# eridgd/WCT-TF

Measured on AMD Instinct MI355X. Metric: stylized frames/sec @512x512, 5-level relu5->1 pipeline, alpha=0.8, higher is better.
Workload: dtype f16

## Files before the change

wct_tf_amd/csrc/stats_gemm.hip:

```cpp
#include "wct_stages.h"


struct StatArgs {
  const float* x[2];
  int n[2];
  const float* u[2];
  const unsigned* umax[2];
  const float* mean;
  float* partial;
  float* absmax;
  int C, nslab;
  int shared_style;
};

__global__ __launch_bounds__(256) void colsum_kernel(StatArgs p) {
  __shared__ f32x4 red[256];
  const int mat = blockIdx.y, slab = blockIdx.x;
  if (skip_style_mat(mat, p.shared_style)) return;
  const int b = mat & 1, pair = mat >> 1;
  const int C = p.C, cq = C / 4;
  const int nrp = 256 / cq;
  const int tid = threadIdx.x;
  const int rp = tid / cq, c4 = tid % cq;
  const int N = p.n[b];
// ... 367 lines not shown
#pragma unroll
      for (int i = 0; i < TM; ++i)
#pragma unroll
        for (int j = 0; j < TM; ++j) {
          acc[i][j] = __builtin_amdgcn_mfma_f32_32x32x16_f16(al[i], bhf[j], acc[i][j], 0, 0, 0);
          acc[i][j] = __builtin_amdgcn_mfma_f32_32x32x16_f16(ah[i], blf[j], acc[i][j], 0, 0, 0);
          acc[i][j] = __builtin_amdgcn_mfma_f32_32x32x16_f16(ah[i], bhf[j], acc[i][j], 0, 0, 0);
        }
    }
  };

  float ra[KPT], rb[KPT];
  if (diag) {
    if (kbeg < kend) load(ra, voff_a, kbeg);
    for (int k0 = kbeg; k0 < kend; k0 += 32) {
      if (k0 + 32 <= kend) split_store(ra, mean_a, k0, false, lds[0], lds[1]);
      else split_store(ra, mean_a, k0, true, lds[0], lds[1]);
      __syncthreads();
      if (k0 + 32 < kend) load(ra, voff_a, k0 + 32);
      mma_stage(lds[0], lds[1]);
      __syncthreads();
    }
  } else {
    if (kbeg < kend) { load(ra, voff_a, kbeg); load(rb, voff_b, kbeg); }
    for (int k0 = kbeg; k0 < kend; k0 += 32) {
      if (k0 + 32 <= kend) {
        split_store(ra, mean_a, k0, false, lds[0], lds[1]);
        split_store(rb, mean_b, k0, false, lds[2], lds[3]);
      } else {
        split_store(ra, mean_a, k0, true, lds[0], lds[1]);
        split_store(rb, mean_b, k0, true, lds[2], lds[3]);
      }
      __syncthreads();
      if (k0 + 32 < kend) { load(ra, voff_a, k0 + 32); load(rb, voff_b, k0 + 32); }
      mma_stage(lds[2], lds[3]);
      __syncthreads();
    }
  }

  float* out = p.partial + ((size_t)mat * p.nsplit + split) * C * C;
#pragma unroll
  for (int i = 0; i < TM; ++i)
#pragma unroll
    for (int j = 0; j < TM; ++j) {
      const int gn = n0 + (wn * TM + j) * 32 + (lane & 31);
#pragma unroll
      for (int r = 0; r < 16; ++r) {
        const int gm = m0 + (wm * TM + i) * 32 + (r & 3) + 8 * (r >> 2) + 4 * (lane >> 5);
        if (gm < C && gn < C) out[(size_t)gm * C + gn] = acc[i][j][r];
      }
    }
}

__global__ __launch_bounds__(256) void cov_finish_kernel(const float* partial, const float* scale, float* cov, int C, int nsplit, int BT,
                                                         float inv0, float inv1, float eps, int shared_style, float* cov0 = nullptr) {
  __shared__ float tt[64][65];
  const int mat = blockIdx.z;
  if (skip_style_mat(mat, shared_style)) return;
  const size_t cc = (size_t)C * C;
  const int r0 = blockIdx.y * 64, c0 = blockIdx.x * 64, tid = threadIdx.x, ty = tid >> 4, tx = tid & 15;
  const bool mirror = r0 / BT > c0 / BT;
  const float* pb = partial + (size_t)mat * nsplit * cc;
  const float sc = scale[mat];
  const float f = ((mat & 1) == 0 ? inv0 : inv1) / (sc * sc);
  f32x4 acc[4];
#pragma unroll
  for (int i = 0; i < 4; ++i) {
    const int r = (mirror ? c0 : r0) + ty * 4 + i, c = (mirror ? r0 : c0) + tx * 4;
    f32x4 sum = {0.f, 0.f, 0.f, 0.f};
    if (r < C && c < C)
      for (int k = 0; k < nsplit; ++k) sum += *reinterpret_cast<const f32x4*>(pb + (size_t)k * cc + (size_t)r * C + c);
    acc[i] = sum;
  }
  if (mirror) {
#pragma unroll
    for (int i = 0; i < 4; ++i)
#pragma unroll
      for (int j = 0; j < 4; ++j) tt[ty * 4 + i][tx * 4 + j] = acc[i][j];
    __syncthreads();
#pragma unroll
    for (int i = 0; i < 4; ++i)
#pragma unroll
      for (int j = 0; j < 4; ++j) acc[i][j] = tt[tx * 4 + j][ty * 4 + i];
  }
#pragma unroll
  for (int i = 0; i < 4; ++i) {
    const int r = r0 + ty * 4 + i, c = c0 + tx * 4;
    if (r >= C || c >= C) continue;
    f32x4 v = acc[i] * f;
#pragma unroll
    for (int j = 0; j < 4; ++j) if (r == c + j) v[j] += eps;
    *reinterpret_cast<f32x4*>(cov + (size_t)mat * cc + (size_t)r * C + c) = v;
    if (cov0) *reinterpret_cast<f32x4*>(cov0 + (size_t)mat * cc + (size_t)r * C + c) = v;
  }
}

int launch_means(const float* content, int Nc, const float* style, int Ns, int C, int P,
                        const WctCarve& w, bool with_var, int shared_style, hipStream_t s, const WctFeatStats* fs) {
  StatArgs sa;
  sa.x[0] = content; sa.x[1] = style; sa.n[0] = Nc; sa.n[1] = Ns;
  for (int b = 0; b < 2; ++b) {
    sa.u[b] = fs && fs->umax[b] ? fs->u[b] : nullptr;
    sa.umax[b] = sa.u[b] ? fs->umax[b] : nullptr;
  }
  sa.mean = nullptr; sa.partial = w.stat_partial; sa.absmax = w.absmax; sa.C = C; sa.nslab = w.nslab; sa.shared_style = shared_style;
  hipLaunchKernelGGL(colsum_kernel, dim3(w.nslab, 2 * P), dim3(256), 0, s, sa);
  hipLaunchKernelGGL(colsum_finish_kernel, dim3(cdiv(C, 256), 2 * P), dim3(256), 0, s, w.stat_partial, w.mean, C, w.nslab, (float)Nc, (float)Ns, shared_style,
                     (const float*)w.absmax, w.scale);
  if (with_var) {
    sa.mean = w.mean; sa.absmax = nullptr;
    hipLaunchKernelGGL(colsum_kernel, dim3(w.nslab, 2 * P), dim3(256), 0, s, sa);
    hipLaunchKernelGGL(colsum_finish_kernel, dim3(cdiv(C, 256), 2 * P), dim3(256), 0, s, w.stat_partial, w.var, C, w.nslab, (float)Nc, (float)Ns, shared_style,
                       (const float*)nullptr, (float*)nullptr);
  }
  HIP_TRY(hipGetLastError());
  return WCT_OK;
}

int launch_cov(const float* content, int Nc, const float* style, int Ns, int C, int P, const WctCarve& w, float eps, int shared_style,
               hipStream_t s) {
  const int BT = C >= 128 ? 128 : 64;
  {
    CovArgs ca;
    ca.x[0] = content; ca.x[1] = style; ca.n[0] = Nc; ca.n[1] = Ns;
    ca.mean = w.mean; ca.scale = w.scale; ca.partial = w.cov_partial;
    ca.C = C; ca.ksplit = w.ksplit; ca.nsplit = w.nsplit; ca.ntile = cdiv(C, BT); ca.shared_style = shared_style;
    dim3 grid(ca.ntile * (ca.ntile + 1) / 2, w.nsplit, 2 * P);
    if (BT == 128) hipLaunchKernelGGL((cov_f16x2_kernel<128>), grid, dim3(256), 0, s, ca);
    else hipLaunchKernelGGL((cov_f16x2_kernel<64>), grid, dim3(256), 0, s, ca);
    HIP_TRY(hipGetLastError());
  }
  hipLaunchKernelGGL(cov_finish_kernel, dim3(cdiv(C, 64), cdiv(C, 64), 2 * P), dim3(256), 0, s, w.cov_partial, w.scale, w.A, C,
                     w.nsplit, BT, 1.f / (float)(Nc - 1), 1.f / (float)(Ns - 1), eps, shared_style, w.A0);
  HIP_TRY(hipGetLastError());
  return WCT_OK;
}

static int launch_slot_means(const float* x, int N, int C, int m, int nslab, const WctCarve& w, bool with_var, hipStream_t s,
                             const float* u = nullptr, const unsigned* umax = nullptr) {
  StatArgs sa = {};
  sa.x[0] = sa.x[1] = x; sa.n[0] = sa.n[1] = N;
  sa.u[0] = umax ? u : nullptr; sa.umax[0] = sa.u[0] ? umax : nullptr;
  float* partial = w.stat_partial + (size_t)m * w.nslab * C;
  float* absmax = w.absmax + (size_t)m * w.nslab;
  sa.mean = nullptr; sa.partial = partial; sa.absmax = absmax; sa.C = C; sa.nslab = nslab; sa.shared_style = 0;
  hipLaunchKernelGGL(colsum_kernel, dim3(nslab, 1), dim3(256), 0, s, sa);
  hipLaunchKernelGGL(colsum_finish_kernel, dim3(cdiv(C, 256), 1), dim3(256), 0, s, partial, w.mean + (size_t)m * C, C, nslab, (float)N,
                     (float)N, 0, (const float*)absmax, w.scale + m);
  if (with_var) {
    sa.mean = w.mean + (size_t)m * C; sa.absmax = nullptr;
    hipLaunchKernelGGL(colsum_kernel, dim3(nslab, 1), dim3(256), 0, s, sa);
    hipLaunchKernelGGL(colsum_finish_kernel, dim3(cdiv(C, 256), 1), dim3(256), 0, s, partial, w.var + (size_t)m * C, C, nslab, (float)N,
                       (float)N, 0, (const float*)nullptr, (float*)nullptr);
  }
  HIP_TRY(hipGetLastError());
  return WCT_OK;
}

static int launch_slot_cov(const float* x, int N, int C, int m, int nsplit, int ksplit, float eps, const WctCarve& w, hipStream_t s) {
  const int BT = C >= 128 ? 128 : 64;
  const size_t cc = (size_t)C * C;
  CovArgs ca;
  ca.x[0] = ca.x[1] = x; ca.n[0] = ca.n[1] = N;
  ca.mean = w.mean + (size_t)m * C; ca.scale = w.scale + m; ca.partial = w.cov_partial + (size_t)m * w.nsplit * cc;
  ca.C = C; ca.ksplit = ksplit; ca.nsplit = nsplit; ca.ntile = cdiv(C, BT); ca.shared_style = 0;
  dim3 grid(ca.ntile * (ca.ntile + 1) / 2, nsplit, 1);
  if (BT == 128) hipLaunchKernelGGL((cov_f16x2_kernel<128>), grid, dim3(256), 0, s, ca);
  else hipLaunchKernelGGL((cov_f16x2_kernel<64>), grid, dim3(256), 0, s, ca);
  hipLaunchKernelGGL(cov_finish_kernel, dim3(cdiv(C, 64), cdiv(C, 64), 1), dim3(256), 0, s,
                     ca.partial, ca.scale, w.A + m * cc, C, nsplit, BT, 1.f / (float)(N - 1), 1.f / (float)(N - 1), eps, 0, w.A0 + m * cc);
  HIP_TRY(hipGetLastError());
  return WCT_OK;
}

int launch_plan_stats(const SlotPlan& sp, int C, bool with_var, bool with_cov, float eps, hipStream_t s) {
  int rc;
  for (int m = 0; m < 2 * sp.P; ++m) {
    const SlotPlan::Slot& t = sp.slot[m];
    if (!t.n) continue;
    if ((rc = launch_slot_means(t.x, t.n, C, m, t.lay.nslab, sp.w, with_var, s, m ? nullptr : sp.u0, m ? nullptr : sp.umax0))) return rc;
    if (with_cov && (rc = launch_slot_cov(t.x, t.n, C, m, t.lay.nsplit, t.lay.ksplit, eps, sp.w, s))) return rc;
  }
  return WCT_OK;
}
```

wct_tf_amd/csrc/wct.hip:

```cpp
#include "wct_stages.h"
#include "jacobi_dev.h"
#include <algorithm>
#include <type_traits>



template <int BC, int BP, typename Args = ApplyArgs>
__global__ __launch_bounds__(256, 2) void apply_f16x2_kernel(Args p) {
  constexpr bool SEGB = std::is_same<Args, ApplySegBatchArgs>::value;
  constexpr bool SEG = std::is_same<Args, ApplySegArgs>::value || SEGB;
  constexpr int TM = BC / 64, TN = BP / 64;
  constexpr int MI = BC * 4 / 256, XI = BP * 4 / 256;
  __shared__ __attribute__((aligned(16))) unsigned char lm[2][BC * 64];
  __shared__ __attribute__((aligned(16))) unsigned char lx[2][BP * 64];
  typedef unsigned int u32x4 __attribute__((ext_vector_type(4)));
  const int tid = threadIdx.x, lane = tid & 63, wave = tid >> 6;
  const int wm = wave >> 1, wn = wave & 1;
  const int pair = blockIdx.z;
  const int n0 = blockIdx.x * BP, c0 = blockIdx.y * BC;
  int seg0 = 0, N = p.N;
  [[maybe_unused]] int row0 = 0;
  if constexpr (SEGB) {
    const int f = seg_frame(p.fl[pair]), lab = seg_label(p.fl[pair]);
    const int first = p.seg_off[f * (WCT_MIX_MAX + 1) + lab];
    N = p.seg_off[f * (WCT_MIX_MAX + 1) + lab + 1] - first;
    if (n0 >= N) return;
    row0 = f * p.N;
    seg0 = row0 + first;
  } else if constexpr (SEG) {
    seg0 = p.seg_off[p.lab[pair]];
    N = p.seg_off[p.lab[pair] + 1] - seg0;
    if (n0 >= N) return;
  }
  const int C = p.C;
  const float* x = p.x + (SEG ? (size_t)seg0 * C : (size_t)pair * N * C);
  const float* M = p.M + (size_t)pair * C * C;
  const float* mean = p.mean + (size_t)pair * 2 * C;
  const float sx = p.xscale[2 * pair];
  float sM = 1.f;
  {
    const float m = __uint_as_float(p.mabs[pair]);
    if (m > 0.f) { int e; frexpf(m, &e); sM = ldexpf(1.f, 14 - e); }
  }

  const float* mp[MI]; const float* xp[XI];
  int moff[MI], xoff[XI], xk[XI];
#pragma unroll
  for (int i = 0; i < MI; ++i) {
    const int item = tid + i * 256, row = item >> 2, kq = item & 3;
    mp[i] = M + (size_t)min(c0 + row, C - 1) * C + kq * 8;
    moff[i] = (row * 4 + (kq ^ ((row >> 2) & 3))) * 16;
  }
#pragma unroll
  for (int i = 0; i < XI; ++i) {
    const int item = tid + i * 256, row = item >> 2, kq = item & 3;
    xp[i] = x + (size_t)min(n0 + row, N - 1) * C + kq * 8;
    xoff[i] = (row * 4 + (kq ^ ((row >> 2) & 3))) * 16;
    xk[i] = kq * 8;
  }

  f32x16 acc[TM][TN];
#pragma unroll
  for (int i = 0; i < TM; ++i)
#pragma unroll
    for (int j = 0; j < TN; ++j)
#pragma unroll
      for (int r = 0; r < 16; ++r) acc[i][j][r] = 0.f;

  f32x4 rm[MI][2], rx[XI][2];
  auto load = [&](int k0) {
#pragma unroll
    for (int i = 0; i < MI; ++i) {
      rm[i][0] = *reinterpret_cast<const f32x4*>(mp[i] + k0);
      rm[i][1] = *reinterpret_cast<const f32x4*>(mp[i] + k0 + 4);
    }
#pragma unroll
    for (int i = 0; i < XI; ++i) {
      rx[i][0] = *reinterpret_cast<const f32x4*>(xp[i] + k0) - *reinterpret_cast<const f32x4*>(mean + k0 + xk[i]);
      rx[i][1] = *reinterpret_cast<const f32x4*>(xp[i] + k0 + 4) - *reinterpret_cast<const f32x4*>(mean + k0 + xk[i] + 4);
    }
  };
  auto split_store = [&](const f32x4 (&r)[2], float sc, unsigned char* hi, unsigned char* lo, int off) {
    half8 h, l;
#pragma unroll
    for (int j = 0; j < 8; ++j) {
      const float v = r[j >> 2][j & 3] * sc;
      h[j] = (half_t)v;
      l[j] = (half_t)(v - (float)h[j]);
    }
    *reinterpret_cast<half8*>(hi + off) = h;
    *reinterpret_cast<half8*>(lo + off) = l;
  };

  load(0);
  for (int k0 = 0; k0 < C; k0 += 32) {
#pragma unroll
    for (int i = 0; i < MI; ++i) split_store(rm[i], sM, lm[0], lm[1], moff[i]);
#pragma unroll
    for (int i = 0; i < XI; ++i) split_store(rx[i], sx, lx[0], lx[1], xoff[i]);
    __syncthreads();
    if (k0 + 32 < C) load(k0 + 32);
#pragma unroll
    for (int ks = 0; ks < 2; ++ks) {
      const int chunk = ks * 2 + (lane >> 5);
      half8 ah[TM], al[TM], bh[TN], bl[TN];
#pragma unroll
      for (int i = 0; i < TM; ++i) {
        const int r = (wm * TM + i) * 32 + (lane & 31);
        const int off = (r * 4 + (chunk ^ ((r >> 2) & 3))) * 16;
        ah[i] = *reinterpret_cast<const half8*>(lm[0] + off);
        al[i] = *reinterpret_cast<const half8*>(lm[1] + off);
      }
#pragma unroll
      for (int j = 0; j < TN; ++j) {
        const int r = (wn * TN + j) * 32 + (lane & 31);
        const int off = (r * 4 + (chunk ^ ((r >> 2) & 3))) * 16;
        bh[j] = *reinterpret_cast<const half8*>(lx[0] + off);
        bl[j] = *reinterpret_cast<const half8*>(lx[1] + off);
      }
#pragma unroll
      for (int i = 0; i < TM; ++i)
#pragma unroll
        for (int j = 0; j < TN; ++j) {
          acc[i][j] = __builtin_amdgcn_mfma_f32_32x32x16_f16(al[i], bh[j], acc[i][j], 0, 0, 0);
          acc[i][j] = __builtin_amdgcn_mfma_f32_32x32x16_f16(ah[i], bl[j], acc[i][j], 0, 0, 0);
          acc[i][j] = __builtin_amdgcn_mfma_f32_32x32x16_f16(ah[i], bh[j], acc[i][j], 0, 0, 0);
        }
    }
    __syncthreads();
  }

  const float inv = 1.f / (sx * sM);
  const float* bias = p.bias + (size_t)pair * C;
  const int kgrp = lane >> 5;
  f32x4 bvs[TM][4];
#pragma unroll
  for (int i = 0; i < TM; ++i)
#pragma unroll
    for (int rq = 0; rq < 4; ++rq) {
      const int co = c0 + (wm * TM + i) * 32 + 8 * rq + 4 * kgrp;
      const f32x4 z = {0.f, 0.f, 0.f, 0.f};
      bvs[i][rq] = co < C ? *reinterpret_cast<const f32x4*>(bias + co) : z;
    }
  int dst[TN];
  if constexpr (SEG)
#pragma unroll
    for (int j = 0; j < TN; ++j) {
      const int n = n0 + (wn * TN + j) * 32 + (lane & 31);
      dst[j] = p.perm[seg0 + (n < N ? n : 0)];
      if constexpr (SEGB) dst[j] += row0;
    }
#pragma unroll
  for (int j = 0; j < TN; ++j) {
    const int n = n0 + (wn * TN + j) * 32 + (lane & 31);
    const bool n_ok = n < N;
    const size_t row = SEG ? (size_t)dst[j] * C : ((size_t)pair * N + (n_ok ? n : 0)) * C;
#pragma unroll
    for (int i = 0; i < TM; ++i) {
      const int cb = c0 + (wm * TM + i) * 32;
      unsigned pk[4][2];
#pragma unroll
      for (int rq = 0; rq < 4; ++rq) {
        const int co = cb + 8 * rq + 4 * kgrp;
        const f32x4 bv = bvs[i][rq];
        f32x4 v;
#pragma unroll
        for (int q = 0; q < 4; ++q) v[q] = acc[i][j][rq * 4 + q] * inv + bv[q];
        if (p.out32 && n_ok && co < C) *reinterpret_cast<f32x4*>(p.out32 + row + co) = v;
        typedef _Float16 h2 __attribute__((ext_vector_type(2)));
        h2 lo = {(half_t)v[0], (half_t)v[1]}, hi = {(half_t)v[2], (half_t)v[3]};
        pk[rq][0] = __builtin_bit_cast(unsigned, lo);
        pk[rq][1] = __builtin_bit_cast(unsigned, hi);
      }
      if (p.out16) {
#pragma unroll
        for (int m = 0; m < 2; ++m) {
          auto sxw = __builtin_amdgcn_permlane32_swap(pk[2 * m][0], pk[2 * m + 1][0], false, false);
          auto syw = __builtin_amdgcn_permlane32_swap(pk[2 * m][1], pk[2 * m + 1][1], false, false);
          u32x4 o = {sxw[0], syw[0], sxw[1], syw[1]};
          const int co = cb + 16 * m + 8 * kgrp;
          if (n_ok && co < C) *reinterpret_cast<u32x4*>(p.out16 + row + co) = o;
        }
      }
    }
  }
}

int launch_apply_seg(const ApplySegArgs& a, int nmax, int P, hipStream_t s) {
  const int C = a.C;
  if (C >= 128) hipLaunchKernelGGL((apply_f16x2_kernel<128, 128, ApplySegArgs>), dim3(cdiv(nmax, 128), cdiv(C, 128), P), dim3(256), 0, s, a);
  else hipLaunchKernelGGL((apply_f16x2_kernel<64, 128, ApplySegArgs>), dim3(cdiv(nmax, 128), cdiv(C, 64), P), dim3(256), 0, s, a);
  HIP_TRY(hipGetLastError());
  return WCT_OK;
}

int launch_apply_seg_batch(const ApplySegBatchArgs& a, int nmax, int P, hipStream_t s) {
  const int C = a.C;
  if (C >= 128) hipLaunchKernelGGL((apply_f16x2_kernel<128, 128, ApplySegBatchArgs>), dim3(cdiv(nmax, 128), cdiv(C, 128), P), dim3(256), 0, s, a);
  else hipLaunchKernelGGL((apply_f16x2_kernel<64, 128, ApplySegBatchArgs>), dim3(cdiv(nmax, 128), cdiv(C, 64), P), dim3(256), 0, s, a);
  HIP_TRY(hipGetLastError());
  return WCT_OK;
}

static int wct_nslab(int N) { int s = cdiv(N, 64); return s < 1 ? 1 : (s > 256 ? 256 : s); }

static void cov_split(int C, int Nmax, int P, int* nsplit, int* ksplit) {
  const int nt = C >= 128 ? cdiv(C, 128) : 1;
  const int tiles = nt * (nt + 1) / 2 * P;
  int want = 32 / tiles;
  if (want < 1) want = 1;
  int ks = cdiv(cdiv(Nmax, want), 32) * 32;
  if (ks < 256) ks = 256;
  *ksplit = ks;
  *nsplit = cdiv(Nmax, ks);
}

PairLayout pair_layout(int C, int Nc, int Ns) {
  PairLayout L;
  const int Nmax = Nc > Ns ? Nc : Ns;
  L.nslab = wct_nslab(Nmax);
  cov_split(C, Nmax, 1, &L.nsplit, &L.ksplit);
  return L;
}

WctCarve carve(void* base, int C, int P, const PairLayout& lay) {
  WctCarve w;
  w.nslab = lay.nslab; w.nsplit = lay.nsplit; w.ksplit = lay.ksplit;
  size_t off = 0;
  char* b = reinterpret_cast<char*>(base);
  auto take = [&](size_t bytes) { void* p = b ? b + off : nullptr; off += align_up(bytes); return p; };
  const size_t cc = (size_t)C * C * sizeof(float);
  w.mean = (float*)take((size_t)2 * P * C * sizeof(float));
  w.var = (float*)take((size_t)2 * P * C * sizeof(float));
  w.stat_partial = (float*)take((size_t)2 * P * w.nslab * C * sizeof(float));
  w.absmax = (float*)take((size_t)2 * P * w.nslab * sizeof(float));
  w.scale = (float*)take((size_t)2 * P * sizeof(float));
  w.cov_partial = (float*)take((size_t)2 * P * w.nsplit * cc);
  w.A = (float*)take(2 * P * cc);
  w.A0 = (float*)take(2 * P * cc);
  w.refresh = (int*)take((size_t)2 * P * sizeof(int));
  w.V = (float*)take(2 * P * cc);
  w.d = (float*)take((size_t)2 * P * C * sizeof(float));
  w.G = (float*)take(2 * P * cc);
  w.X = (float*)take(2 * P * cc);
  w.S2 = (float*)take(7 * P * cc);
  w.Tw = (float*)take(2 * P * cc);
  w.Tcs = w.Tw + (size_t)C * C;
  w.T = (float*)take(P * cc);
  w.M = (float*)take(P * cc);
  w.bias = (float*)take((size_t)P * C * sizeof(float));
  w.mabs = (unsigned*)take((size_t)P * sizeof(unsigned));
  w.jacobi_bytes = jacobi_workspace_bytes(C, 2 * P) + 4 * (1024 + 64 * sizeof(JacobiState));
  w.jacobi_ws = take(w.jacobi_bytes);
  w.mix = (float*)take((size_t)2 * C * sizeof(float));
  w.total = off;
  return w;
}

size_t wct_workspace_bytes(int C, int Nc, int Ns, int P) {
  const int Cw = C < 32 ? 32 : C;
  return carve(nullptr, Cw, P, pair_layout(Cw, Nc, Ns)).total;
}

int launch_blend(const WctCarve& w, int C, int P, float alpha, int shared_style, hipStream_t s) {
  const size_t cc = (size_t)C * C;
  GemmArgs g = {};
  g.A = w.Tcs; g.lda = C; g.a_kmajor = 0; g.B = w.Tw; g.ldb = C; g.b_kmajor = 1; g.sA = shared_style ? 0 : 2 * cc; g.sB = 2 * cc;
  g.M = C; g.N = C; g.K = C; g.ksplit = C; g.out32 = w.M; g.ldo = C; g.s_out = cc;
  g.blend = 1; g.alpha = alpha; g.mabs = w.mabs;
  return launch_gemm(g, 1, P, s);
}

static int launch_blend_apply(const WctCarve& w, const float* content, int Nc, int C, int P, float alpha, int shared_style,
                              half_t* out16, float* out32, hipStream_t s) {
  int rc;
  if ((rc = launch_blend(w, C, P, alpha, shared_style, s))) return rc;
  {
    ApplyArgs a;
    a.x = content; a.N = Nc; a.C = C; a.mean = w.mean; a.M = w.M; a.bias = w.bias;
    a.xscale = w.scale; a.mabs = w.mabs; a.out16 = out16; a.out32 = out32;
    if (C >= 128) hipLaunchKernelGGL((apply_f16x2_kernel<128, 128>), dim3(cdiv(Nc, 128), cdiv(C, 128), P), dim3(256), 0, s, a);
    else hipLaunchKernelGGL((apply_f16x2_kernel<64, 128>), dim3(cdiv(Nc, 128), cdiv(C, 64), P), dim3(256), 0, s, a);
  }
  HIP_TRY(hipGetLastError());
  return WCT_OK;
}

WctStyleKey wct_style_key(int C, int Nc, int Ns) {
  const PairLayout L = pair_layout(std::max(C, 32), Nc, Ns);
  return WctStyleKey{L.nslab, L.nsplit, L.ksplit};
}
size_t wct_style_state_floats(int C) { return (size_t)2 * C + (size_t)C * C; }

template <typename Ref>
__global__ __launch_bounds__(256) void style_load_kernel(Ref r, float* mean, float* var, float* Tw, int C, int with_T) {
  const int k = blockIdx.y;
  const float* src = r.state[k];
  const size_t cc = (size_t)C * C, n = (size_t)2 * C + (with_T ? cc : 0), slot = (size_t)(2 * k + 1);
  for (size_t i = (blockIdx.x * (size_t)blockDim.x + threadIdx.x) * 4; i < n; i += (size_t)gridDim.x * blockDim.x * 4) {
    const f32x4 v = *reinterpret_cast<const f32x4*>(src + i);
    float* dst = i < (size_t)C ? mean + slot * C + i : (i < (size_t)2 * C ? var + slot * C + (i - C) : Tw + slot * cc + (i - 2 * C));
    *reinterpret_cast<f32x4*>(dst) = v;
  }
}

static int launch_style_load(const WctStyleRef& r, int K, const WctCarve& w, int C, bool with_T, hipStream_t s) {
  for (int k = 0; k < K; ++k) ARG_CHECK(r.state[k] != nullptr);
  const size_t n4 = ((size_t)2 * C + (with_T ? (size_t)C * C : 0)) / 4;
  hipLaunchKernelGGL(style_load_kernel<WctStyleRef>, dim3((unsigned)std::min<size_t>((n4 + 255) / 256, 256), K), dim3(256), 0, s, r, w.mean,
                     w.var, w.Tw, C, with_T ? 1 : 0);
  HIP_TRY(hipGetLastError());
  return WCT_OK;
}

int launch_style_load_slots(const WctStyleSlots& r, int P, const WctCarve& w, int C, bool with_T, hipStream_t s) {
  ARG_CHECK(P >= 1 && P <= WCT_PLAN_PAIRS);
  for (int p = 0; p < P; ++p) ARG_CHECK(r.state[p] != nullptr);
  const size_t n4 = ((size_t)2 * C + (with_T ? (size_t)C * C : 0)) / 4;
  hipLaunchKernelGGL(style_load_kernel<WctStyleSlots>, dim3((unsigned)std::min<size_t>((n4 + 255) / 256, 256), P), dim3(256), 0, s, r, w.mean,
                     w.var, w.Tw, C, with_T ? 1 : 0);
  HIP_TRY(hipGetLastError());
  return WCT_OK;
}

static void style_plan(SlotPlan* sp, void* base, int C, const float* style, int Ns, const WctStyleKey& key) {
  *sp = SlotPlan{};
  sp->P = 1; sp->skip = WCT_SKIP_CONTENT; sp->nwhite = 0;
  sp->slot[1] = {style, Ns, PairLayout{key.nslab, key.nsplit, key.ksplit}};
  plan_carve(sp, base, C);
}

size_t wct_style_workspace_bytes(int C, int Ns, const WctStyleKey& key) {
  SlotPlan sp;
  style_plan(&sp, nullptr, C, nullptr, Ns, key);
  return sp.total;
}

int launch_style_state(const float* style, int Ns, int C, const WctStyleKey& key, int adain, int mode, float eps_in, void* workspace,
// ... 224 lines not shown
```

wct_tf_amd/csrc/wct_stages.h:

```cpp
#pragma once
#include "common.h"

constexpr int WCT_SKIP_MIX = 2;
constexpr int WCT_SKIP_STYLE = 3, WCT_SKIP_CONTENT = 4, WCT_SKIP_MIX_STYLE = 5;
constexpr int WCT_SKIP_STYLES = 6;
__device__ __host__ __forceinline__ bool skip_style_mat(int mat, int shared_style) {
  if (shared_style >= WCT_SKIP_STYLE)
    return shared_style == WCT_SKIP_STYLE ? (mat & 1) != 0
                                          : (shared_style == WCT_SKIP_CONTENT ? (mat & 1) == 0
                                                                              : (shared_style == WCT_SKIP_MIX_STYLE ? mat > 0 : (mat & 1) != 0));
  return shared_style == WCT_SKIP_MIX ? ((mat & 1) == 0 && mat > 0) : (shared_style && (mat & 1) && mat > 1);
}
__device__ __host__ __forceinline__ bool one_content(int shared_style) { return shared_style == WCT_SKIP_MIX || shared_style == WCT_SKIP_MIX_STYLE; }
__device__ __host__ __forceinline__ bool one_style(int shared_style) { return shared_style == 1 || shared_style == WCT_SKIP_STYLE; }

constexpr int EIG_CORRECT = 2;
constexpr float JACOBI_TOL_FN = 1.5e-2f;
constexpr float JACOBI_TOL_FN2 = 4e-2f;
constexpr float JACOBI_TOL_FN_WCT = EIG_CORRECT >= 2 ? JACOBI_TOL_FN2 : (EIG_CORRECT ? JACOBI_TOL_FN : 0.f);

static inline size_t align_up(size_t x) { return (x + 255) & ~(size_t)255; }

struct WctCarve {
  float *mean, *var, *stat_partial, *absmax, *scale, *cov_partial, *A, *A0, *V, *d, *G, *X, *S2, *Tw, *Tcs, *T, *M, *bias, *mix;
  unsigned* mabs; int* refresh;
  void* jacobi_ws; size_t jacobi_bytes;
  int nslab, nsplit, ksplit;
  size_t total;
};

struct PairLayout { int nslab, nsplit, ksplit; };
PairLayout pair_layout(int C, int Nc, int Ns);
WctCarve carve(void* base, int C, int P, const PairLayout& lay);

static inline float cov_eps(int mode, float eps_in) {
  return mode == WCT_MODE_TF ? (eps_in >= 0.f ? eps_in : 1e-8f) : 0.f;
}

static inline unsigned rows_grid(size_t N, int C) {
  const size_t blocks = (N * C / 4 + 255) / 256;
  return (unsigned)(blocks > 2048 ? 2048 : blocks);
}

constexpr int WCT_PLAN_PAIRS = 32;
struct SlotPlan {
  int P, skip, nwhite;
  struct Slot { const float* x; int n; PairLayout lay; } slot[2 * WCT_PLAN_PAIRS];
  const float* u0; const unsigned* umax0;
  WctCarve w;
  size_t total;
};
void plan_carve(SlotPlan* sp, void* base, int C);
bool plan_fits(const SlotPlan& sp, int C);

struct ApplyArgs {
  const float* x; int N; int C;
  const float* mean;
  const float* M; const float* bias;
  const float* xscale;
  const unsigned* mabs;
  half_t* out16; float* out32;
};
struct ApplySegArgs : ApplyArgs { const int* seg_off; const int* perm; int lab[WCT_MIX_MAX]; };
struct ApplySegBatchArgs : ApplyArgs { const int* seg_off; const int* perm; unsigned char fl[WCT_PLAN_PAIRS]; };
__device__ __host__ __forceinline__ int seg_frame(unsigned char fl) { return fl >> 3; }
__device__ __host__ __forceinline__ int seg_label(unsigned char fl) { return fl & 7; }

int launch_means(const float* content, int Nc, const float* style, int Ns, int C, int P, const WctCarve& w, bool with_var,
                 int shared_style, hipStream_t s, const WctFeatStats* fs = nullptr);
int launch_cov(const float* content, int Nc, const float* style, int Ns, int C, int P, const WctCarve& w, float eps, int shared_style,
               hipStream_t s);
int launch_plan_stats(const SlotPlan& sp, int C, bool with_var, bool with_cov, float eps, hipStream_t s);
int launch_eig_stage(const WctCarve& w, int C, int P, int skip, int u_f16, int* sweeps_dev, int* eig_fail, hipStream_t s,
                     int check_from = 2);
int launch_refresh(const WctCarve& w, int C, int P, int shared_style, hipStream_t s, bool always = false);
int launch_spectral_tail(const WctCarve& w, int C, int P, float alpha, int mode, float eps_in, int shared_style, int nwhite, hipStream_t s);
int launch_spectral_function(const float* A, const float* V, float* G, float* X, float* out, int C, int nbatch, size_t stride,
                             size_t out_stride, int kind, float shift, hipStream_t s, float* scratch2 = nullptr);
int launch_blend(const WctCarve& w, int C, int P, float alpha, int shared_style, hipStream_t s);
int launch_apply_seg(const ApplySegArgs& a, int nmax, int P, hipStream_t s);
int launch_apply_seg_batch(const ApplySegBatchArgs& a, int nmax, int P, hipStream_t s);
int launch_warm_rotate(const WctCarve& w, int C, int P, const float* V0, hipStream_t s);
int launch_warm_compose(const WctCarve& w, int C, int P, const float* V0, hipStream_t s);
int launch_warm_store(const float* V, float* scratch, float* basis, int C, hipStream_t s);
int launch_style_load_slots(const WctStyleSlots& r, int P, const WctCarve& w, int C, bool with_T, hipStream_t s);
```

Measured before the change: 664.0.

## Add 256-wide 512-thread tiles for covariance and apply GEMMs on large C

After: 665.8, median of 6. About the same (+0.3%).

```diff
diff --git a/wct_tf_amd/csrc/stats_gemm.hip b/wct_tf_amd/csrc/stats_gemm.hip
--- a/wct_tf_amd/csrc/stats_gemm.hip
+++ b/wct_tf_amd/csrc/stats_gemm.hip
@@ -443,6 +443,151 @@
     }
 }
 
+constexpr int COV_WIDE = 256;
+constexpr int COV_WIDE_LDS = 2 * 4 * COV_WIDE * 64;
+
+__global__ __launch_bounds__(512, 1) void cov_f16x2_wide_kernel(CovArgs p) {
+  constexpr int BT = COV_WIDE, TM = 4, TN = 2, PLANE = BT * 64;
+  extern __shared__ __attribute__((aligned(16))) unsigned char cov_lds[];
+  typedef unsigned int u32x4 __attribute__((ext_vector_type(4)));
+  const int tid = threadIdx.x, lane = tid & 63, wave = __builtin_amdgcn_readfirstlane(tid >> 6);
+  const int wm = wave >> 2, wn = wave & 3;
+  int ti = 0, rem = blockIdx.x;
+  while (rem >= p.ntile - ti) { rem -= p.ntile - ti; ++ti; }
+  const int tj = ti + rem;
+  const bool diag = ti == tj;
+  const int m0 = ti * BT, n0 = tj * BT;
+  const int mat = blockIdx.z, split = blockIdx.y;
+  if (skip_style_mat(mat, p.shared_style)) return;
+  const int side = mat & 1, pair = mat >> 1;
+  const int N = p.n[side], C = p.C;
+  const float* x = p.x[side] + (size_t)pair * N * C;
+  const int kbeg = split * p.ksplit;
+  const int kend = min(N, kbeg + p.ksplit);
+  const float sc = p.scale[mat];
+
+  const int op = wave >> 2, kg = wave & 3;
+  const bool stager = !(diag && op);
+  const int cq = min((op ? n0 : m0) + lane * 4, C - 4);
+  const f32x4 mean4 = *reinterpret_cast<const f32x4*>(p.mean + mat * C + cq);
+  const __amdgpu_buffer_rsrc_t rsrc = __builtin_amdgcn_make_buffer_rsrc((void*)x, 0, (int)((size_t)N * C * 4), 0x00020000);
+  const int voff = cq * 4;
+  const int poff = op * 2 * PLANE;
+
+  f32x16 acc[TM][TN];
+#pragma unroll
+  for (int i = 0; i < TM; ++i)
+#pragma unroll
+    for (int j = 0; j < TN; ++j)
+#pragma unroll
+      for (int r = 0; r < 16; ++r) acc[i][j][r] = 0.f;
+
+  f32x4 rr[8];
+  auto load = [&](int k0) {
+#pragma unroll
+    for (int j = 0; j < 8; ++j)
+      rr[j] = __builtin_bit_cast(f32x4, __builtin_amdgcn_raw_buffer_load_b128(rsrc, voff, (k0 + kg * 8 + j) * C * 4, 0));
+  };
+  auto park = [&](unsigned char* img, int k0) {
+    const bool tail = k0 + 32 > kend;
+#pragma unroll
+    for (int q = 0; q < 4; ++q) {
+      half8 h, l;
+#pragma unroll
+      for (int j = 0; j < 8; ++j) {
+        const float s_in = (!tail || k0 + kg * 8 + j < kend) ? sc : 0.f;
+        const float v = (rr[j][q] - mean4[q]) * s_in;
+        h[j] = (half_t)v;
+        l[j] = (half_t)(v - (float)h[j]);
+      }
+      const int c = lane * 4 + q;
+      const int off = (c * 4 + (kg ^ (lane & 3))) * 16;
+      *reinterpret_cast<half8*>(img + poff + off) = h;
+      *reinterpret_cast<half8*>(img + poff + PLANE + off) = l;
+    }
+  };
+  const bool below = diag && wm == 1 && wn < 2;
+  const int boff = diag ? 0 : 2 * PLANE;
+
+  if (stager && kbeg < kend) { load(kbeg); park(cov_lds, kbeg); }
+  __syncthreads();
+  int st = 0;
+  for (int k0 = kbeg; k0 < kend; k0 += 32, st ^= 1) {
+    const unsigned char* img = cov_lds + st * (4 * PLANE);
+    const bool more = stager && k0 + 32 < kend;
+    if (more) load(k0 + 32);
+    if (!below) {
+#pragma unroll
+      for (int ks = 0; ks < 2; ++ks) {
+        const int chunk = ks * 2 + (lane >> 5);
+        half8 ah[TM], al[TM], bh[TN], bl[TN];
+#pragma unroll
+        for (int i = 0; i < TM; ++i) {
+          const int r = (wm * TM + i) * 32 + (lane & 31);
+          const int off = (r * 4 + (chunk ^ ((r >> 2) & 3))) * 16;
+          ah[i] = *reinterpret_cast<const half8*>(img + off);
+          al[i] = *reinterpret_cast<const half8*>(img + PLANE + off);
+        }
+#pragma unroll
+        for (int j = 0; j < TN; ++j) {
+          const int r = (wn * TN + j) * 32 + (lane & 31);
+          const int off = (r * 4 + (chunk ^ ((r >> 2) & 3))) * 16;
+          bh[j] = *reinterpret_cast<const half8*>(img + boff + off);
+          bl[j] = *reinterpret_cast<const half8*>(img + boff + PLANE + off);
+        }
+#pragma unroll
+        for (int i = 0; i < TM; ++i)
+#pragma unroll
+          for (int j = 0; j < TN; ++j) {
+            acc[i][j] = __builtin_amdgcn_mfma_f32_32x32x16_f16(al[i], bh[j], acc[i][j], 0, 0, 0);
+            acc[i][j] = __builtin_amdgcn_mfma_f32_32x32x16_f16(ah[i], bl[j], acc[i][j], 0, 0, 0);
+            acc[i][j] = __builtin_amdgcn_mfma_f32_32x32x16_f16(ah[i], bh[j], acc[i][j], 0, 0, 0);
+          }
+      }
+    }
+    if (more) park(cov_lds + (st ^ 1) * (4 * PLANE), k0 + 32);
+    __syncthreads();
+  }
+  if (below) return;
+
+  float* out = p.partial + ((size_t)mat * p.nsplit + split) * C * C;
+#pragma unroll
+  for (int i = 0; i < TM; ++i)
+#pragma unroll
+    for (int j = 0; j < TN; ++j) {
+      const int gn = n0 + (wn * TN + j) * 32 + (lane & 31);
+#pragma unroll
+      for (int r = 0; r < 16; ++r) {
+        const int gm = m0 + (wm * TM + i) * 32 + (r & 3) + 8 * (r >> 2) + 4 * (lane >> 5);
+        if (gm < C && gn < C) out[(size_t)gm * C + gn] = acc[i][j][r];
+      }
+    }
+}
+
+static int launch_cov_tiles(CovArgs ca, int nmat, hipStream_t s) {
+  const int C = ca.C, tiles = wct_tail_tiles();
+  const int ntw = cdiv(C, COV_WIDE);
+  if (C >= 256 && tiles && (tiles == 2 || (long)ntw * (ntw + 1) / 2 * ca.nsplit * nmat >= 256)) {
+    static bool raised[16] = {};
+    int dev = 0;
+    HIP_TRY(hipGetDevice(&dev));
+    if (dev >= 0 && dev < 16 && !raised[dev]) {
+      HIP_TRY(hipFuncSetAttribute(reinterpret_cast<const void*>(&cov_f16x2_wide_kernel), hipFuncAttributeMaxDynamicSharedMemorySize, COV_WIDE_LDS));
+      raised[dev] = true;
+    }
+    ca.ntile = ntw;
+    hipLaunchKernelGGL(cov_f16x2_wide_kernel, dim3(ntw * (ntw + 1) / 2, ca.nsplit, nmat), dim3(512), COV_WIDE_LDS, s, ca);
+  } else {
+    const int BT = C >= 128 ? 128 : 64;
+    ca.ntile = cdiv(C, BT);
+    dim3 grid(ca.ntile * (ca.ntile + 1) / 2, ca.nsplit, nmat);
+    if (BT == 128) hipLaunchKernelGGL((cov_f16x2_kernel<128>), grid, dim3(256), 0, s, ca);
+    else hipLaunchKernelGGL((cov_f16x2_kernel<64>), grid, dim3(256), 0, s, ca);
+  }
+  HIP_TRY(hipGetLastError());
+  return WCT_OK;
+}
+
 __global__ __launch_bounds__(256) void cov_finish_kernel(const float* partial, const float* scale, float* cov, int C, int nsplit, int BT,
                                                          float inv0, float inv1, float eps, int shared_style, float* cov0 = nullptr) {
   __shared__ float tt[64][65];
@@ -511,16 +656,12 @@
 int launch_cov(const float* content, int Nc, const float* style, int Ns, int C, int P, const WctCarve& w, float eps, int shared_style,
                hipStream_t s) {
   const int BT = C >= 128 ? 128 : 64;
-  {
-    CovArgs ca;
-    ca.x[0] = content; ca.x[1] = style; ca.n[0] = Nc; ca.n[1] = Ns;
-    ca.mean = w.mean; ca.scale = w.scale; ca.partial = w.cov_partial;
-    ca.C = C; ca.ksplit = w.ksplit; ca.nsplit = w.nsplit; ca.ntile = cdiv(C, BT); ca.shared_style = shared_style;
-    dim3 grid(ca.ntile * (ca.ntile + 1) / 2, w.nsplit, 2 * P);
-    if (BT == 128) hipLaunchKernelGGL((cov_f16x2_kernel<128>), grid, dim3(256), 0, s, ca);
-    else hipLaunchKernelGGL((cov_f16x2_kernel<64>), grid, dim3(256), 0, s, ca);
-    HIP_TRY(hipGetLastError());
-  }
+  int rc;
+  CovArgs ca;
+  ca.x[0] = content; ca.x[1] = style; ca.n[0] = Nc; ca.n[1] = Ns;
+  ca.mean = w.mean; ca.scale = w.scale; ca.partial = w.cov_partial;
+  ca.C = C; ca.ksplit = w.ksplit; ca.nsplit = w.nsplit; ca.shared_style = shared_style;
+  if ((rc = launch_cov_tiles(ca, 2 * P, s))) return rc;
   hipLaunchKernelGGL(cov_finish_kernel, dim3(cdiv(C, 64), cdiv(C, 64), 2 * P), dim3(256), 0, s, w.cov_partial, w.scale, w.A, C,
                      w.nsplit, BT, 1.f / (float)(Nc - 1), 1.f / (float)(Ns - 1), eps, shared_style, w.A0);
   HIP_TRY(hipGetLastError());
@@ -554,10 +695,9 @@
   CovArgs ca;
   ca.x[0] = ca.x[1] = x; ca.n[0] = ca.n[1] = N;
   ca.mean = w.mean + (size_t)m * C; ca.scale = w.scale + m; ca.partial = w.cov_partial + (size_t)m * w.nsplit * cc;
-  ca.C = C; ca.ksplit = ksplit; ca.nsplit = nsplit; ca.ntile = cdiv(C, BT); ca.shared_style = 0;
-  dim3 grid(ca.ntile * (ca.ntile + 1) / 2, nsplit, 1);
-  if (BT == 128) hipLaunchKernelGGL((cov_f16x2_kernel<128>), grid, dim3(256), 0, s, ca);
-  else hipLaunchKernelGGL((cov_f16x2_kernel<64>), grid, dim3(256), 0, s, ca);
+  ca.C = C; ca.ksplit = ksplit; ca.nsplit = nsplit; ca.shared_style = 0;
+  int rc;
+  if ((rc = launch_cov_tiles(ca, 1, s))) return rc;
   hipLaunchKernelGGL(cov_finish_kernel, dim3(cdiv(C, 64), cdiv(C, 64), 1), dim3(256), 0, s,
                      ca.partial, ca.scale, w.A + m * cc, C, nsplit, BT, 1.f / (float)(N - 1), 1.f / (float)(N - 1), eps, 0, w.A0 + m * cc);
   HIP_TRY(hipGetLastError());
diff --git a/wct_tf_amd/csrc/wct.hip b/wct_tf_amd/csrc/wct.hip
--- a/wct_tf_amd/csrc/wct.hip
+++ b/wct_tf_amd/csrc/wct.hip
@@ -1,135 +1,62 @@
 #include "wct_stages.h"
 #include "jacobi_dev.h"
 #include <algorithm>
+#include <cstdlib>
 #include <type_traits>
 
 
 
-template <int BC, int BP, typename Args = ApplyArgs>
-__global__ __launch_bounds__(256, 2) void apply_f16x2_kernel(Args p) {
-  constexpr bool SEGB = std::is_same<Args, ApplySegBatchArgs>::value;
-  constexpr bool SEG = std::is_same<Args, ApplySegArgs>::value || SEGB;
-  constexpr int TM = BC / 64, TN = BP / 64;
-  constexpr int MI = BC * 4 / 256, XI = BP * 4 / 256;
-  __shared__ __attribute__((aligned(16))) unsigned char lm[2][BC * 64];
-  __shared__ __attribute__((aligned(16))) unsigned char lx[2][BP * 64];
-  typedef unsigned int u32x4 __attribute__((ext_vector_type(4)));
-  const int tid = threadIdx.x, lane = tid & 63, wave = tid >> 6;
-  const int wm = wave >> 1, wn = wave & 1;
-  const int pair = blockIdx.z;
-  const int n0 = blockIdx.x * BP, c0 = blockIdx.y * BC;
-  int seg0 = 0, N = p.N;
-  [[maybe_unused]] int row0 = 0;
-  if constexpr (SEGB) {
-    const int f = seg_frame(p.fl[pair]), lab = seg_label(p.fl[pair]);
-    const int first = p.seg_off[f * (WCT_MIX_MAX + 1) + lab];
-    N = p.seg_off[f * (WCT_MIX_MAX + 1) + lab + 1] - first;
-    if (n0 >= N) return;
-    row0 = f * p.N;
-    seg0 = row0 + first;
-  } else if constexpr (SEG) {
-    seg0 = p.seg_off[p.lab[pair]];
-    N = p.seg_off[p.lab[pair] + 1] - seg0;
-    if (n0 >= N) return;
-  }
-  const int C = p.C;
-  const float* x = p.x + (SEG ? (size_t)seg0 * C : (size_t)pair * N * C);
-  const float* M = p.M + (size_t)pair * C * C;
-  const float* mean = p.mean + (size_t)pair * 2 * C;
-  const float sx = p.xscale[2 * pair];
-  float sM = 1.f;
-  {
+template <typename Args>
+struct ApplyBlock {
+  static constexpr bool SEGB = std::is_same<Args, ApplySegBatchArgs>::value;
+  static constexpr bool SEG = std::is_same<Args, ApplySegArgs>::value || SEGB;
+  const float *x, *M, *mean;
+  float sx, sM;
+  int N, seg0 = 0;
+  int row0 = 0;
+  __device__ __forceinline__ ApplyBlock(const Args& p, int pair) {
+    N = p.N;
+    if constexpr (SEGB) {
+      const int f = seg_frame(p.fl[pair]), lab = seg_label(p.fl[pair]);
+      const int first = p.seg_off[f * (WCT_MIX_MAX + 1) + lab];
+      N = p.seg_off[f * (WCT_MIX_MAX + 1) + lab + 1] - first;
+      row0 = f * p.N;
+      seg0 = row0 + first;
+    } else if constexpr (SEG) {
+      seg0 = p.seg_off[p.lab[pair]];
+      N = p.seg_off[p.lab[pair] + 1] - seg0;
+    }
+    const int C = p.C;
+    x = p.x + (SEG ? (size_t)seg0 * C : (size_t)pair * N * C);
+    M = p.M + (size_t)pair * C * C;
+    mean = p.mean + (size_t)pair * 2 * C;
+    sx = p.xscale[2 * pair];
+    sM = 1.f;
     const float m = __uint_as_float(p.mabs[pair]);
     if (m > 0.f) { int e; frexpf(m, &e); sM = ldexpf(1.f, 14 - e); }
   }
-
-  const float* mp[MI]; const float* xp[XI];
-  int moff[MI], xoff[XI], xk[XI];
-#pragma unroll
-  for (int i = 0; i < MI; ++i) {
-    const int item = tid + i * 256, row = item >> 2, kq = item & 3;
-    mp[i] = M + (size_t)min(c0 + row, C - 1) * C + kq * 8;
-    moff[i] = (row * 4 + (kq ^ ((row >> 2) & 3))) * 16;
-  }
-#pragma unroll
-  for (int i = 0; i < XI; ++i) {
-    const int item = tid + i * 256, row = item >> 2, kq = item & 3;
-    xp[i] = x + (size_t)min(n0 + row, N - 1) * C + kq * 8;
-    xoff[i] = (row * 4 + (kq ^ ((row >> 2) & 3))) * 16;
-    xk[i] = kq * 8;
-  }
-
-  f32x16 acc[TM][TN];
-#pragma unroll
-  for (int i = 0; i < TM; ++i)
-#pragma unroll
-    for (int j = 0; j < TN; ++j)
-#pragma unroll
-      for (int r = 0; r < 16; ++r) acc[i][j][r] = 0.f;
-
-  f32x4 rm[MI][2], rx[XI][2];
-  auto load = [&](int k0) {
-#pragma unroll
-    for (int i = 0; i < MI; ++i) {
-      rm[i][0] = *reinterpret_cast<const f32x4*>(mp[i] + k0);
-      rm[i][1] = *reinterpret_cast<const f32x4*>(mp[i] + k0 + 4);
-    }
-#pragma unroll
-    for (int i = 0; i < XI; ++i) {
-      rx[i][0] = *reinterpret_cast<const f32x4*>(xp[i] + k0) - *reinterpret_cast<const f32x4*>(mean + k0 + xk[i]);
-      rx[i][1] = *reinterpret_cast<const f32x4*>(xp[i] + k0 + 4) - *reinterpret_cast<const f32x4*>(mean + k0 + xk[i] + 4);
-    }
-  };
-  auto split_store = [&](const f32x4 (&r)[2], float sc, unsigned char* hi, unsigned char* lo, int off) {
-    half8 h, l;
-#pragma unroll
-    for (int j = 0; j < 8; ++j) {
-      const float v = r[j >> 2][j & 3] * sc;
-      h[j] = (half_t)v;
-      l[j] = (half_t)(v - (float)h[j]);
-    }
-    *reinterpret_cast<half8*>(hi + off) = h;
-    *reinterpret_cast<half8*>(lo + off) = l;
-  };
-
-  load(0);
-  for (int k0 = 0; k0 < C; k0 += 32) {
-#pragma unroll
-    for (int i = 0; i < MI; ++i) split_store(rm[i], sM, lm[0], lm[1], moff[i]);
-#pragma unroll
-    for (int i = 0; i < XI; ++i) split_store(rx[i], sx, lx[0], lx[1], xoff[i]);
-    __syncthreads();
-    if (k0 + 32 < C) load(k0 + 32);
-#pragma unroll
-    for (int ks = 0; ks < 2; ++ks) {
-      const int chunk = ks * 2 + (lane >> 5);
-      half8 ah[TM], al[TM], bh[TN], bl[TN];
-#pragma unroll
-      for (int i = 0; i < TM; ++i) {
-        const int r = (wm * TM + i) * 32 + (lane & 31);
-        const int off = (r * 4 + (chunk ^ ((r >> 2) & 3))) * 16;
-        ah[i] = *reinterpret_cast<const half8*>(lm[0] + off);
-        al[i] = *reinterpret_cast<const half8*>(lm[1] + off);
-      }
-#pragma unroll
-      for (int j = 0; j < TN; ++j) {
-        const int r = (wn * TN + j) * 32 + (lane & 31);
-        const int off = (r * 4 + (chunk ^ ((r >> 2) & 3))) * 16;
-        bh[j] = *reinterpret_cast<const half8*>(lx[0] + off);
-        bl[j] = *reinterpret_cast<const half8*>(lx[1] + off);
-      }
-#pragma unroll
-      for (int i = 0; i < TM; ++i)
-#pragma unroll
-        for (int j = 0; j < TN; ++j) {
-          acc[i][j] = __builtin_amdgcn_mfma_f32_32x32x16_f16(al[i], bh[j], acc[i][j], 0, 0, 0);
-          acc[i][j] = __builtin_amdgcn_mfma_f32_32x32x16_f16(ah[i], bl[j], acc[i][j], 0, 0, 0);
-          acc[i][j] = __builtin_amdgcn_mfma_f32_32x32x16_f16(ah[i], bh[j], acc[i][j], 0, 0, 0);
-        }
-    }
-    __syncthreads();
-  }
-
+};
+
+__device__ __forceinline__ void apply_split_store(const f32x4 (&r)[2], float sc, unsigned char* hi, unsigned char* lo, int off) {
+  half8 h, l;
+#pragma unroll
+  for (int j = 0; j < 8; ++j) {
+    const float v = r[j >> 2][j & 3] * sc;
+    h[j] = (half_t)v;
+    l[j] = (half_t)(v - (float)h[j]);
+  }
+  *reinterpret_cast<half8*>(hi + off) = h;
+  *reinterpret_cast<half8*>(lo + off) = l;
+}
+
+template <int TM, int TN, typename Args>
+__device__ __forceinline__ void apply_store(const Args& p, const ApplyBlock<Args>& b, const f32x16 (&acc)[TM][TN], int pair, int cw,
+                                            int nw, int lane) {
+  constexpr bool SEGB = ApplyBlock<Args>::SEGB, SEG = ApplyBlock<Args>::SEG;
+  typedef unsigned int u32x4 __attribute__((ext_vector_type(4)));
+  const int C = p.C, N = b.N, seg0 = b.seg0;
+  [[maybe_unused]] const int row0 = b.row0;
+  const float sx = b.sx, sM = b.sM;
   const float inv = 1.f / (sx * sM);
   const float* bias = p.bias + (size_t)pair * C;
   const int kgrp = lane >> 5;
@@ -138,7 +65,7 @@
   for (int i = 0; i < TM; ++i)
 #pragma unroll
     for (int rq = 0; rq < 4; ++rq) {
-      const int co = c0 + (wm * TM + i) * 32 + 8 * rq + 4 * kgrp;
+      const int co = cw + i * 32 + 8 * rq + 4 * kgrp;
       const f32x4 z = {0.f, 0.f, 0.f, 0.f};
       bvs[i][rq] = co < C ? *reinterpret_cast<const f32x4*>(bias + co) : z;
     }
@@ -146,18 +73,18 @@
   if constexpr (SEG)
 #pragma unroll
     for (int j = 0; j < TN; ++j) {
-      const int n = n0 + (wn * TN + j) * 32 + (lane & 31);
+      const int n = nw + j * 32 + (lane & 31);
       dst[j] = p.perm[seg0 + (n < N ? n : 0)];
       if constexpr (SEGB) dst[j] += row0;
     }
 #pragma unroll
   for (int j = 0; j < TN; ++j) {
-    const int n = n0 + (wn * TN + j) * 32 + (lane & 31);
+    const int n = nw + j * 32 + (lane & 31);
     const bool n_ok = n < N;
     const size_t row = SEG ? (size_t)dst[j] * C : ((size_t)pair * N + (n_ok ? n : 0)) * C;
 #pragma unroll
     for (int i = 0; i < TM; ++i) {
-      const int cb = c0 + (wm * TM + i) * 32;
+      const int cb = cw + i * 32;
       unsigned pk[4][2];
 #pragma unroll
       for (int rq = 0; rq < 4; ++rq) {
@@ -186,21 +113,228 @@
   }
 }
 
-int launch_apply_seg(const ApplySegArgs& a, int nmax, int P, hipStream_t s) {
-  const int C = a.C;
-  if (C >= 128) hipLaunchKernelGGL((apply_f16x2_kernel<128, 128, ApplySegArgs>), dim3(cdiv(nmax, 128), cdiv(C, 128), P), dim3(256), 0, s, a);
-  else hipLaunchKernelGGL((apply_f16x2_kernel<64, 128, ApplySegArgs>), dim3(cdiv(nmax, 128), cdiv(C, 64), P), dim3(256), 0, s, a);
+template <int BC, int BP, typename Args = ApplyArgs>
+__global__ __launch_bounds__(256, 2) void apply_f16x2_kernel(Args p) {
+  constexpr int TM = BC / 64, TN = BP / 64;
+  constexpr int MI = BC * 4 / 256, XI = BP * 4 / 256;
+  __shared__ __attribute__((aligned(16))) unsigned char lm[2][BC * 64];
+  __shared__ __attribute__((aligned(16))) unsigned char lx[2][BP * 64];
+  const int tid = threadIdx.x, lane = tid & 63, wave = tid >> 6;
+  const int wm = wave >> 1, wn = wave & 1;
+  const int pair = blockIdx.z;
+  const int n0 = blockIdx.x * BP, c0 = blockIdx.y * BC;
+  const ApplyBlock<Args> b(p, pair);
+  if (n0 >= b.N) return;
+  const int N = b.N, C = p.C;
+  const float* x = b.x; const float* M = b.M; const float* mean = b.mean;
+  const float sx = b.sx, sM = b.sM;
+
+  const float* mp[MI]; const float* xp[XI];
+  int moff[MI], xoff[XI], xk[XI];
+#pragma unroll
+  for (int i = 0; i < MI; ++i) {
+    const int item = tid + i * 256, row = item >> 2, kq = item & 3;
+    mp[i] = M + (size_t)min(c0 + row, C - 1) * C + kq * 8;
+    moff[i] = (row * 4 + (kq ^ ((row >> 2) & 3))) * 16;
+  }
+#pragma unroll
+  for (int i = 0; i < XI; ++i) {
+    const int item = tid + i * 256, row = item >> 2, kq = item & 3;
+    xp[i] = x + (size_t)min(n0 + row, N - 1) * C + kq * 8;
+    xoff[i] = (row * 4 + (kq ^ ((row >> 2) & 3))) * 16;
+    xk[i] = kq * 8;
+  }
+
+  f32x16 acc[TM][TN];
+#pragma unroll
+  for (int i = 0; i < TM; ++i)
+#pragma unroll
+    for (int j = 0; j < TN; ++j)
+#pragma unroll
+      for (int r = 0; r < 16; ++r) acc[i][j][r] = 0.f;
+
+  f32x4 rm[MI][2], rx[XI][2];
+  auto load = [&](int k0) {
+#pragma unroll
+    for (int i = 0; i < MI; ++i) {
+      rm[i][0] = *reinterpret_cast<const f32x4*>(mp[i] + k0);
+      rm[i][1] = *reinterpret_cast<const f32x4*>(mp[i] + k0 + 4);
+    }
+#pragma unroll
+    for (int i = 0; i < XI; ++i) {
+      rx[i][0] = *reinterpret_cast<const f32x4*>(xp[i] + k0) - *reinterpret_cast<const f32x4*>(mean + k0 + xk[i]);
+      rx[i][1] = *reinterpret_cast<const f32x4*>(xp[i] + k0 + 4) - *reinterpret_cast<const f32x4*>(mean + k0 + xk[i] + 4);
+    }
+  };
+
+  load(0);
+  for (int k0 = 0; k0 < C; k0 += 32) {
+#pragma unroll
+    for (int i = 0; i < MI; ++i) apply_split_store(rm[i], sM, lm[0], lm[1], moff[i]);
+#pragma unroll
+    for (int i = 0; i < XI; ++i) apply_split_store(rx[i], sx, lx[0], lx[1], xoff[i]);
+    __syncthreads();
+    if (k0 + 32 < C) load(k0 + 32);
+#pragma unroll
+    for (int ks = 0; ks < 2; ++ks) {
+      const int chunk = ks * 2 + (lane >> 5);
+      half8 ah[TM], al[TM], bh[TN], bl[TN];
+#pragma unroll
+      for (int i = 0; i < TM; ++i) {
+        const int r = (wm * TM + i) * 32 + (lane & 31);
+        const int off = (r * 4 + (chunk ^ ((r >> 2) & 3))) * 16;
+        ah[i] = *reinterpret_cast<const half8*>(lm[0] + off);
+        al[i] = *reinterpret_cast<const half8*>(lm[1] + off);
+      }
+#pragma unroll
+      for (int j = 0; j < TN; ++j) {
+        const int r = (wn * TN + j) * 32 + (lane & 31);
+        const int off = (r * 4 + (chunk ^ ((r >> 2) & 3))) * 16;
+        bh[j] = *reinterpret_cast<const half8*>(lx[0] + off);
+        bl[j] = *reinterpret_cast<const half8*>(lx[1] + off);
+      }
+#pragma unroll
+      for (int i = 0; i < TM; ++i)
+#pragma unroll
+        for (int j = 0; j < TN; ++j) {
+          acc[i][j] = __builtin_amdgcn_mfma_f32_32x32x16_f16(al[i], bh[j], acc[i][j], 0, 0, 0);
+          acc[i][j] = __builtin_amdgcn_mfma_f32_32x32x16_f16(ah[i], bl[j], acc[i][j], 0, 0, 0);
+          acc[i][j] = __builtin_amdgcn_mfma_f32_32x32x16_f16(ah[i], bh[j], acc[i][j], 0, 0, 0);
+        }
+    }
+    __syncthreads();
+  }
+
+  apply_store<TM, TN>(p, b, acc, pair, c0 + wm * TM * 32, n0 + wn * TN * 32, lane);
+}
+
+constexpr int APPLY_WIDE = 256;
+constexpr int APPLY_WIDE_LDS = 2 * 4 * APPLY_WIDE * 64;
+
+template <typename Args>
+__global__ __launch_bounds__(512, 1) void apply_f16x2_wide_kernel(Args p) {
+  constexpr int BT = APPLY_WIDE, TM = 4, TN = 2;
+  constexpr int NI = BT * 4 / 512;
+  constexpr int PLANE = BT * 64;
+  extern __shared__ __attribute__((aligned(16))) unsigned char apply_lds[];
+  const int tid = threadIdx.x, lane = tid & 63, wave = tid >> 6;
+  const int wm = wave >> 2, wn = wave & 3;
+  const int pair = blockIdx.z;
+  const int n0 = blockIdx.x * BT, c0 = blockIdx.y * BT;
+  const ApplyBlock<Args> b(p, pair);
+  if (n0 >= b.N) return;
+  const int N = b.N, C = p.C;
+  const float* mean = b.mean;
+  const float sx = b.sx, sM = b.sM;
+
+  const float* mp[NI]; const float* xp[NI];
+  int soff[NI], sk[NI];
+#pragma unroll
+  for (int i = 0; i < NI; ++i) {
+    const int item = tid + i * 512, row = item >> 2, kq = item & 3;
+    mp[i] = b.M + (size_t)min(c0 + row, C - 1) * C + kq * 8;
+    xp[i] = b.x + (size_t)min(n0 + row, N - 1) * C + kq * 8;
+    soff[i] = (row * 4 + (kq ^ ((row >> 2) & 3))) * 16;
+    sk[i] = kq * 8;
+  }
+
+  f32x16 acc[TM][TN];
+#pragma unroll
+  for (int i = 0; i < TM; ++i)
+#pragma unroll
+    for (int j = 0; j < TN; ++j)
+#pragma unroll
+      for (int r = 0; r < 16; ++r) acc[i][j][r] = 0.f;
+
+  f32x4 rm[NI][2], rx[NI][2];
+  auto load = [&](int k0) {
+#pragma unroll
+    for (int i = 0; i < NI; ++i) {
+      rm[i][0] = *reinterpret_cast<const f32x4*>(mp[i] + k0);
+      rm[i][1] = *reinterpret_cast<const f32x4*>(mp[i] + k0 + 4);
+      rx[i][0] = *reinterpret_cast<const f32x4*>(xp[i] + k0) - *reinterpret_cast<const f32x4*>(mean + k0 + sk[i]);
+      rx[i][1] = *reinterpret_cast<const f32x4*>(xp[i] + k0 + 4) - *reinterpret_cast<const f32x4*>(mean + k0 + sk[i] + 4);
+    }
+  };
+  auto park = [&](unsigned char* img) {
+#pragma unroll
+    for (int i = 0; i < NI; ++i) {
+      apply_split_store(rm[i], sM, img, img + PLANE, soff[i]);
+      apply_split_store(rx[i], sx, img + 2 * PLANE, img + 3 * PLANE, soff[i]);
+    }
+  };
+
+  load(0);
+  park(apply_lds);
+  __syncthreads();
+  int st = 0;
+  for (int k0 = 0; k0 < C; k0 += 32, st ^= 1) {
+    const unsigned char* img = apply_lds + st * (4 * PLANE);
+    const bool more = k0 + 32 < C;
+    if (more) load(k0 + 32);
+#pragma unroll
+    for (int ks = 0; ks < 2; ++ks) {
+      const int chunk = ks * 2 + (lane >> 5);
+      half8 ah[TM], al[TM], bh[TN], bl[TN];
+#pragma unroll
+      for (int i = 0; i < TM; ++i) {
+        const int r = (wm * TM + i) * 32 + (lane & 31);
+        const int off = (r * 4 + (chunk ^ ((r >> 2) & 3))) * 16;
+        ah[i] = *reinterpret_cast<const half8*>(img + off);
+        al[i] = *reinterpret_cast<const half8*>(img + PLANE + off);
+      }
+#pragma unroll
+      for (int j = 0; j < TN; ++j) {
+        const int r = (wn * TN + j) * 32 + (lane & 31);
+        const int off = (r * 4 + (chunk ^ ((r >> 2) & 3))) * 16;
+        bh[j] = *reinterpret_cast<const half8*>(img + 2 * PLANE + off);
+        bl[j] = *reinterpret_cast<const half8*>(img + 3 * PLANE + off);
+      }
+#pragma unroll
+      for (int i = 0; i < TM; ++i)
+#pragma unroll
+        for (int j = 0; j < TN; ++j) {
+          acc[i][j] = __builtin_amdgcn_mfma_f32_32x32x16_f16(al[i], bh[j], acc[i][j], 0, 0, 0);
+          acc[i][j] = __builtin_amdgcn_mfma_f32_32x32x16_f16(ah[i], bl[j], acc[i][j], 0, 0, 0);
+          acc[i][j] = __builtin_amdgcn_mfma_f32_32x32x16_f16(ah[i], bh[j], acc[i][j], 0, 0, 0);
+        }
+    }
+    if (more) park(apply_lds + (st ^ 1) * (4 * PLANE));
+    __syncthreads();
+  }
+  apply_store<TM, TN>(p, b, acc, pair, c0 + wm * TM * 32, n0 + wn * TN * 32, lane);
+}
+
+int wct_tail_tiles() {
+  static const int v = getenv("WCT_TAIL_TILES") ? atoi(getenv("WCT_TAIL_TILES")) : 1;
+  return v;
+}
+
+template <typename Args>
+static int launch_apply_tiles(const Args& a, int nmax, int P, hipStream_t s) {
+  const int C = a.C, tiles = wct_tail_tiles();
+  const long wide_blocks = (long)cdiv(nmax, APPLY_WIDE) * cdiv(C, APPLY_WIDE) * P;
+  if (C >= 256 && tiles && (tiles == 2 || (C >= 512 && wide_blocks >= 256))) {
+    static bool raised[16] = {};
+    int dev = 0;
+    HIP_TRY(hipGetDevice(&dev));
+    if (dev >= 0 && dev < 16 && !raised[dev]) {
+      HIP_TRY(hipFuncSetAttribute(reinterpret_cast<const void*>(&apply_f16x2_wide_kernel<Args>), hipFuncAttributeMaxDynamicSharedMemorySize,
+                                  APPLY_WIDE_LDS));
+      raised[dev] = true;
+    }
+    hipLaunchKernelGGL((apply_f16x2_wide_kernel<Args>), dim3(cdiv(nmax, APPLY_WIDE), cdiv(C, APPLY_WIDE), P), dim3(512), APPLY_WIDE_LDS, s, a);
+  } else if (C >= 128) {
+    hipLaunchKernelGGL((apply_f16x2_kernel<128, 128, Args>), dim3(cdiv(nmax, 128), cdiv(C, 128), P), dim3(256), 0, s, a);
+  } else {
+    hipLaunchKernelGGL((apply_f16x2_kernel<64, 128, Args>), dim3(cdiv(nmax, 128), cdiv(C, 64), P), dim3(256), 0, s, a);
+  }
   HIP_TRY(hipGetLastError());
   return WCT_OK;
 }
 
-int launch_apply_seg_batch(const ApplySegBatchArgs& a, int nmax, int P, hipStream_t s) {
-  const int C = a.C;
-  if (C >= 128) hipLaunchKernelGGL((apply_f16x2_kernel<128, 128, ApplySegBatchArgs>), dim3(cdiv(nmax, 128), cdiv(C, 128), P), dim3(256), 0, s, a);
-  else hipLaunchKernelGGL((apply_f16x2_kernel<64, 128, ApplySegBatchArgs>), dim3(cdiv(nmax, 128), cdiv(C, 64), P), dim3(256), 0, s, a);
-  HIP_TRY(hipGetLastError());
-  return WCT_OK;
-}
+int launch_apply_seg(const ApplySegArgs& a, int nmax, int P, hipStream_t s) { return launch_apply_tiles(a, nmax, P, s); }
+int launch_apply_seg_batch(const ApplySegBatchArgs& a, int nmax, int P, hipStream_t s) { return launch_apply_tiles(a, nmax, P, s); }
 
 static int wct_nslab(int N) { int s = cdiv(N, 64); return s < 1 ? 1 : (s > 256 ? 256 : s); }
 
@@ -275,15 +409,10 @@
                               half_t* out16, float* out32, hipStream_t s) {
   int rc;
   if ((rc = launch_blend(w, C, P, alpha, shared_style, s))) return rc;
-  {
-    ApplyArgs a;
-    a.x = content; a.N = Nc; a.C = C; a.mean = w.mean; a.M = w.M; a.bias = w.bias;
-    a.xscale = w.scale; a.mabs = w.mabs; a.out16 = out16; a.out32 = out32;
-    if (C >= 128) hipLaunchKernelGGL((apply_f16x2_kernel<128, 128>), dim3(cdiv(Nc, 128), cdiv(C, 128), P), dim3(256), 0, s, a);
-    else hipLaunchKernelGGL((apply_f16x2_kernel<64, 128>), dim3(cdiv(Nc, 128), cdiv(C, 64), P), dim3(256), 0, s, a);
-  }
-  HIP_TRY(hipGetLastError());
-  return WCT_OK;
+  ApplyArgs a;
+  a.x = content; a.N = Nc; a.C = C; a.mean = w.mean; a.M = w.M; a.bias = w.bias;
+  a.xscale = w.scale; a.mabs = w.mabs; a.out16 = out16; a.out32 = out32;
+  return launch_apply_tiles(a, Nc, P, s);
 }
 
 WctStyleKey wct_style_key(int C, int Nc, int Ns) {
diff --git a/wct_tf_amd/csrc/wct_stages.h b/wct_tf_amd/csrc/wct_stages.h
--- a/wct_tf_amd/csrc/wct_stages.h
+++ b/wct_tf_amd/csrc/wct_stages.h
@@ -53,6 +53,8 @@
 void plan_carve(SlotPlan* sp, void* base, int C);
 bool plan_fits(const SlotPlan& sp, int C);
 
+int wct_tail_tiles();
+
 struct ApplyArgs {
   const float* x; int N; int C;
   const float* mean;
```
